# ak110/object_detector

Hardware: AMD Instinct MI355X
Metric: images_per_sec (higher is better)
Workload: dtype f16

## Files before the change

### object_detector_amd/csrc/detect.hip

```cpp
#include <string.h>

#include "post_common.h"

namespace {

constexpr int NB = OD_TOPK_NB;
constexpr int DT_ROWS = OD_DT_ROWS, DT2_RPT = OD_DT2_RPT;
constexpr int DT_CAND_CAP = 1024;

__global__ __launch_bounds__(256) void od_detect_pass1(const float* __restrict__ pred, const float* __restrict__ priors,
                                                       float* __restrict__ boxes, float* __restrict__ rowmax,
                                                       float* __restrict__ conf_out, int* __restrict__ hist,
                                                       TopkState* __restrict__ st, int P, int NC, float loc_scale, int clip,
                                                       float thr, unsigned dbase, int dshift) {
  extern __shared__ __attribute__((aligned(16))) float sm[];
  const int C = NC + 6, tid = threadIdx.x, b = blockIdx.y;
  float* rows = sm;
  int* lh = (int*)(sm + DT_ROWS * C);
  const int p0 = blockIdx.x * DT_ROWS;
  const int nrows = min(DT_ROWS, P - p0);
  for (int i = tid; i < NB; i += 256) lh[i] = 0;
  if (blockIdx.x == 0 && tid == 0) {
    TopkState z = {0, 0, 0, 0};
    st[b] = z;
  }
  const long long r0 = (long long)b * P + p0;
  const float* src = pred + r0 * C;
  const int nel = nrows * C;
  for (int i = tid * 4; i < nel; i += 256 * 4) {
    if (i + 3 < nel) {
      *(f32x4*)(rows + i) = *(const f32x4*)(src + i);
    } else {
      for (int e = i; e < nel; ++e) rows[e] = src[e];
    }
  }
  __syncthreads();
  if (tid < nrows) {
    float* row = rows + tid * C;
    const f32x4 loc = {row[2 + NC], row[3 + NC], row[4 + NC], row[5 + NC]};
    od_row_conf(row, NC, row + 2);
    float mx = 0.f;
    for (int c = 0; c < NC; ++c) {
      const float v = row[2 + c];
      mx = fmaxf(mx, v);
      const unsigned sb = od_score_bits(v, thr);
      if (sb) atomicAdd(&lh[od_digit0(sb, dbase, dshift)], 1);
    }
    rowmax[r0 + tid] = mx;
    const f32x4 pr = *(const f32x4*)(priors + (long long)(p0 + tid) * 4);
    *(f32x4*)(boxes + (r0 + tid) * 4) = od_decode_one(loc, pr, loc_scale, clip);
  }
  __syncthreads();
  int* gh = hist + (long long)b * NB;
  for (int i = tid; i < NB; i += 256)
    if (lh[i]) atomicAdd(&gh[i], lh[i]);
  if (conf_out) {
    float* dst = conf_out + r0 * NC;
    for (int i = tid; i < nrows * NC; i += 256) {
      const int r = i / NC, c = i - r * NC;
      dst[i] = rows[r * C + 2 + c];
    }
  }
}

__global__ __launch_bounds__(256) void od_detect_pass2(const float* __restrict__ pred, const float* __restrict__ rowmax,
                                                       const int* __restrict__ hist, TopkState* __restrict__ st,
                                                       u64* __restrict__ keys, u64* __restrict__ cand, int P, int NC, int K,
                                                       float thr, long long cand_stride, unsigned dbase, int dshift) {
  extern __shared__ __attribute__((aligned(16))) float sm[];
  const int C = NC + 6, tid = threadIdx.x, b = blockIdx.y;
  float* rows = sm;
  u64* l_out = (u64*)(sm + DT_ROWS * C);
  u64* l_cand = l_out + K;
  __shared__ int n_out, n_cand, n_hot, base_out, base_cand, sh_fd[8];
  __shared__ int hot_list[DT_ROWS * DT2_RPT];
  if (tid == 0) {
    n_out = 0;
    n_cand = 0;
    n_hot = 0;
  }
  int d0, above;
  od_find_digit_256(hist + (long long)b * NB, K, sh_fd, &d0, &above);
  if (blockIdx.x == 0 && tid == 0) {
    st[b].d0 = d0;
    st[b].krem = d0 < 0 ? 0 : K - above;
  }
  const int p_base = blockIdx.x * (DT_ROWS * DT2_RPT);
  const int nh = od_compact_hot_priors(rowmax + (long long)b * P, P, p_base, thr, dbase, dshift, d0, hot_list, &n_hot);
  for (int e = tid; e < nh; e += 256) {
    const int p = hot_list[e];
    float* row = rows + tid * C;
    const float* src = pred + ((long long)b * P + p) * C;
    for (int c = 0; c < 2 + NC; ++c) row[c] = src[c];
    od_row_conf(row, NC, row + 2);
    for (int c = 0; c < NC; ++c) {
      const unsigned sbc = od_score_bits(row[2 + c], thr);
      if (!sbc) continue;
      const int dg = od_digit0(sbc, dbase, dshift);
      if (dg < d0) continue;
      const unsigned flat = (unsigned)(p * NC + c);
      const u64 key = od_make_key(sbc, flat);
      if (dg > d0) {
        l_out[atomicAdd(&n_out, 1)] = key;
      } else {
        const int slot = atomicAdd(&n_cand, 1);
        if (slot < DT_CAND_CAP) {
          l_cand[slot] = key;
        } else {
          cand[(long long)b * cand_stride + atomicAdd(&st[b].ncand, 1)] = key;
        }
      }
    }
  }
  __syncthreads();
  const int nc = min(n_cand, DT_CAND_CAP);
  if (tid == 0) base_cand = nc ? atomicAdd(&st[b].ncand, nc) : 0;
  od_block_copy_out(l_out, n_out, &st[b].nout, keys + (long long)b * K, &base_out);
  u64* oc = cand + (long long)b * cand_stride + base_cand;
  for (int j = tid; j < nc; j += 256) oc[j] = l_cand[j];
}

__global__ __launch_bounds__(1024) void od_detect_refine_sort(const float* __restrict__ boxes, TopkState* __restrict__ st,
                                                              u64* __restrict__ keys, const u64* __restrict__ cand,
                                                              int* __restrict__ hist, int* __restrict__ counts, int P, int NC,
                                                              int K, int KP, long long cand_stride, u64* __restrict__ skeys,
                                                              f32x4* __restrict__ sbox, int* __restrict__ scls, unsigned dbase,
                                                              int dshift) {
  __shared__ u64 s[1024];
  __shared__ int n_win;
  const int b = blockIdx.x, tid = threadIdx.x;
  const TopkState t = st[b];
  const int nout0 = min(t.nout, K);
  if (tid == 0) n_win = 0;
  s[tid] = tid < nout0 ? keys[(long long)b * K + tid] : 0ull;
  __syncthreads();
  if (t.d0 >= 0 && t.krem > 0) {
    const u64* ic = cand + (long long)b * cand_stride;
    od_radix_refine(
        t.ncand, t.ncand, t.krem, dbase, dshift, [&](int i) { return ic[i]; },
        [&](u64 key) {
          const int slot = nout0 + atomicAdd(&n_win, 1);
          if (slot < K) s[slot] = key;
        });
    __syncthreads();
  }
  od_bitonic_sort_desc(s, KP);
  od_rank_gather(s, min(nout0 + n_win, K), b, boxes, P, NC, K, KP, skeys, sbox, scls, keys, counts, hist);
}

__global__ __launch_bounds__(256) void od_gather_det_pred(const float* __restrict__ pred, const float* __restrict__ boxes,
                                                          const int32_t* __restrict__ keep_flat,
                                                          const int32_t* __restrict__ keep_count, int P, int NC, int max_det,
                                                          float* __restrict__ out) {
  extern __shared__ __attribute__((aligned(16))) float sm[];
  const int b = blockIdx.x, C = NC + 6;
  const int n = keep_count[b];
  float* o = out + (size_t)b * (1 + 6 * (size_t)max_det);
  if (threadIdx.x == 0) o[0] = __int_as_float(n);
  float* row = sm + threadIdx.x * C;
  for (int r = threadIdx.x; r < max_det; r += 256) {
    float* rec = o + 1 + 6 * (size_t)r;
    if (r < n) {
      const int flat = keep_flat[(size_t)b * max_det + r];
      const int p = flat / NC, c = flat - p * NC;
      const float* src = pred + ((size_t)b * P + p) * C;
      for (int e = 0; e < 2 + NC; ++e) row[e] = src[e];
      od_row_conf(row, NC, row + 2);
      const float* bx = boxes + ((size_t)b * P + p) * 4;
      rec[0] = __int_as_float(flat);
      rec[1] = row[2 + c];
      rec[2] = bx[0];
      rec[3] = bx[1];
      rec[4] = bx[2];
      rec[5] = bx[3];
    } else {
      rec[0] = __int_as_float(-1);
      rec[1] = rec[2] = rec[3] = rec[4] = rec[5] = 0.f;
    }
  }
}

struct DetLayout {
  size_t hist, state, rowmax, cand, total;
  long long cand_stride;
  size_t nhot, hot;
};
DetLayout det_layout(int B, int P, int NC) {
  DetLayout l;
  size_t o = 0;
  l.hist = o;
  o += (size_t)B * NB * sizeof(int);
  l.state = o;
  o += ((size_t)B * sizeof(TopkState) + 255) & ~(size_t)255;
  l.rowmax = o;
  o += (((size_t)B * P * sizeof(float)) + 255) & ~(size_t)255;
  if (NC > OD_MAX_LDS_NC) {
    l.cand = 0;
    l.cand_stride = 0;
    l.nhot = o;
    o += ((size_t)B * sizeof(int) + 255) & ~(size_t)255;
    l.hot = o;
    o += (size_t)B * P * sizeof(HotRow);
    l.total = o;
    return l;
  }
  l.nhot = l.hot = 0;
  l.cand = o;
  l.cand_stride = (long long)P * NC;
  o += (size_t)B * (size_t)l.cand_stride * sizeof(u64);
  l.total = o;
  return l;
}

}

extern "C" size_t od_detect_workspace_bytes(int B, int P, int NC, int K) {
  (void)K;
  if (B <= 0 || P <= 0 || NC <= 0) return 0;
  return det_layout(B, P, NC).total;
}

extern "C" int od_detect_workspace_init(od_ctx* ctx, void* workspace, size_t workspace_bytes, int B, int P, int NC, void* stream) {
  OD_REQUIRE(ctx && workspace && B > 0 && P > 0 && NC > 0, "od_detect_workspace_init: bad argument");
  const DetLayout l = det_layout(B, P, NC);
  if (workspace_bytes < l.total) {
    od_set_error("od_detect_workspace_init: workspace %zu < %zu bytes", workspace_bytes, l.total);
    return OD_ERR_WORKSPACE;
  }
  OD_CHECK_HIP(hipMemsetAsync(workspace, 0, l.rowmax, (hipStream_t)stream));
  return OD_OK;
}

namespace {
int detect_candidates_launch(od_ctx* ctx, const char* who, const float* pred, const float* priors, int B, int P, int NC,
                             float loc_scale, int clip, float conf_threshold, int K, float* boxes, float* conf, uint64_t* keys,
                             int32_t* counts, void* workspace, size_t workspace_bytes, void* nms_workspace,
                             size_t nms_workspace_bytes, hipStream_t s) {
  OD_REQUIRE(NC >= 1 && NC <= OD_MAX_NC, "%s: NC = %d outside the supported class counts 1..%d", who, NC, OD_MAX_NC);
  OD_REQUIRE(B > 0 && B <= 65535 && P > 0 && P % 2 == 0 && K > 0 && K <= 1024, "%s: bad dims (P even, K <= 1024)", who);
  OD_REQUIRE((long long)P * NC < (1LL << 31), "%s: P * NC must fit 31 bits", who);
  OD_REQUIRE(conf_threshold >= 0.f, "%s: conf_threshold must be >= 0 (scores are probabilities)", who);
  const DetLayout l = det_layout(B, P, NC);
  if (workspace_bytes < l.total) {
    od_set_error("%s: workspace %zu < %zu bytes", who, workspace_bytes, l.total);
    return OD_ERR_WORKSPACE;
  }
  if (nms_workspace_bytes < od_nms_workspace_bytes(B, K)) {
    od_set_error("%s: NMS workspace %zu < %zu bytes", who, nms_workspace_bytes, od_nms_workspace_bytes(B, K));
    return OD_ERR_WORKSPACE;
  }
  char* ws = (char*)workspace;
  int* hist = (int*)(ws + l.hist);
  TopkState* st = (TopkState*)(ws + l.state);
  float* rowmax = (float*)(ws + l.rowmax);
  u64* cand = (u64*)(ws + l.cand);
  const int C = NC + 6;
  unsigned dbase;
  memcpy(&dbase, &conf_threshold, 4);
  int dshift = 0;
  while (((0x3F800000u - dbase) >> dshift) >= (unsigned)NB) ++dshift;
  const dim3 grid((unsigned)od_ceil_div(P, DT_ROWS), (unsigned)B);
  const dim3 grid2((unsigned)od_ceil_div(P, DT_ROWS * DT2_RPT), (unsigned)B);
  u64* skeys;
  f32x4* sbox;
  int* scls;
  int KP;
  od_nms_sorted_buffers(nms_workspace, B, K, &skeys, &sbox, &scls, &KP);
  if (NC > OD_MAX_LDS_NC) {
    return od_detect_wide_launch(pred, priors, B, P, NC, loc_scale, clip, conf_threshold, dbase, dshift, K, KP, boxes, conf,
                                 (u64*)keys, counts, hist, st, rowmax, (int*)(ws + l.nhot), (HotRow*)(ws + l.hot), skeys, sbox,
                                 scls, s);
  }
  const size_t lds1 = (size_t)DT_ROWS * C * 4 + (size_t)NB * 4;
  if (int rc = od_ensure_lds(ctx, (const void*)&od_detect_pass1, lds1)) return rc;
  hipLaunchKernelGGL(od_detect_pass1, grid, dim3(256), lds1, s, pred, priors, boxes, rowmax, conf, hist, st, P, NC, loc_scale,
                     clip, conf_threshold, dbase, dshift);
  OD_CHECK_LAUNCH();
  const size_t lds2 = (size_t)DT_ROWS * C * 4 + ((size_t)K + DT_CAND_CAP) * 8;
  if (int rc = od_ensure_lds(ctx, (const void*)&od_detect_pass2, lds2)) return rc;
  hipLaunchKernelGGL(od_detect_pass2, grid2, dim3(256), lds2, s, pred, rowmax, hist, st, (u64*)keys, cand, P, NC, K,
                     conf_threshold, l.cand_stride, dbase, dshift);
  OD_CHECK_LAUNCH();
  hipLaunchKernelGGL(od_detect_refine_sort, dim3(B), dim3(1024), 0, s, boxes, st, (u64*)keys, cand, hist, counts, P, NC, K, KP,
                     l.cand_stride, skeys, sbox, scls, dbase, dshift);
  OD_CHECK_LAUNCH();
  return OD_OK;
}
}

extern "C" int od_detect(od_ctx* ctx, const float* pred, const float* priors, int B, int P, int NC, float loc_scale, int clip,
                         float conf_threshold, int K, float iou_threshold, int strict, int max_det, float* boxes, float* conf,
                         uint64_t* keys, int32_t* counts, int32_t* keep_flat, int32_t* keep_count, void* workspace,
                         size_t workspace_bytes, void* nms_workspace, size_t nms_workspace_bytes, void* stream) {
  OD_REQUIRE(ctx && pred && priors && boxes && keys && counts && keep_flat && keep_count && workspace && nms_workspace,
             "od_detect: null argument");
  OD_REQUIRE(max_det > 0, "od_detect: bad dims (P even, K <= 1024)");
  hipStream_t s = (hipStream_t)stream;
  if (int rc = detect_candidates_launch(ctx, "od_detect", pred, priors, B, P, NC, loc_scale, clip, conf_threshold, K, boxes, conf,
                                        keys, counts, workspace, workspace_bytes, nms_workspace, nms_workspace_bytes, s))
    return rc;
  return od_nms_mask_scan_launch(ctx, nms_workspace, counts, B, K, iou_threshold, strict, max_det, keep_flat, keep_count, s);
}

extern "C" int od_detect_candidates(od_ctx* ctx, const float* pred, const float* priors, int B, int P, int NC, float loc_scale,
                                    int clip, float conf_threshold, int K, float* boxes, float* conf, uint64_t* keys,
                                    int32_t* counts, void* workspace, size_t workspace_bytes, void* nms_workspace,
                                    size_t nms_workspace_bytes, void* stream) {
  OD_REQUIRE(ctx && pred && priors && boxes && keys && counts && workspace && nms_workspace, "od_detect_candidates: null argument");
  return detect_candidates_launch(ctx, "od_detect_candidates", pred, priors, B, P, NC, loc_scale, clip, conf_threshold, K, boxes,
                                  conf, keys, counts, workspace, workspace_bytes, nms_workspace, nms_workspace_bytes,
                                  (hipStream_t)stream);
}

extern "C" int od_gather_detections_pred(od_ctx* ctx, const float* pred, const float* boxes, const int32_t* keep_flat,
                                         const int32_t* keep_count, int B, int P, int NC, int max_det, float* out, void* stream) {
  OD_REQUIRE(ctx && pred && boxes && keep_flat && keep_count && out, "od_gather_detections_pred: null argument");
  OD_REQUIRE(NC >= 1 && NC <= OD_MAX_NC, "od_gather_detections_pred: NC = %d outside the supported class counts 1..%d", NC,
             OD_MAX_NC);
  OD_REQUIRE(B > 0 && P > 0 && max_det > 0, "od_gather_detections_pred: bad dims");
  if (NC > OD_MAX_LDS_NC) {
    return od_gather_det_pred_wide_launch(pred, boxes, keep_flat, keep_count, B, P, NC, max_det, out, (hipStream_t)stream);
  }
  hipLaunchKernelGGL(od_gather_det_pred, dim3(B), dim3(256), (size_t)256 * (NC + 6) * 4, (hipStream_t)stream, pred, boxes,
                     keep_flat, keep_count, P, NC, max_det, out);
  OD_CHECK_LAUNCH();
  return OD_OK;
}
```

### object_detector_amd/csrc/nms.hip

```cpp
#include "post_common.h"

namespace {

__global__ __launch_bounds__(1024) void od_nms_sort(const float* __restrict__ boxes, const u64* __restrict__ keys,
                                                    const int* __restrict__ counts, int P, int NC, int K, int KP,
                                                    u64* __restrict__ skeys, f32x4* __restrict__ sbox,
                                                    int* __restrict__ scls) {
  __shared__ u64 s[1024];
  const int b = blockIdx.x, tid = threadIdx.x;
  if (tid < KP) s[tid] = tid < K ? keys[(long long)b * K + tid] : 0ull;
  __syncthreads();
  od_bitonic_sort_desc(s, KP);
  od_rank_gather(s, counts[b], b, boxes, P, NC, K, KP, skeys, sbox, scls, nullptr, nullptr, nullptr);
}

__global__ __launch_bounds__(1024) void od_nms_mask(const f32x4* __restrict__ sbox, const int* __restrict__ scls,
                                                   const int* __restrict__ counts, int KP, int W, float thr, int strict,
                                                   u64* __restrict__ mask) {
  extern __shared__ __attribute__((aligned(16))) char sm[];
  f32x4* lb = (f32x4*)sm;
  int* lc = (int*)(sm + (size_t)KP * 16);
  const int b = blockIdx.y, rb = blockIdx.x, tid = threadIdx.x, lane = tid & 63, wv = tid >> 6;
  const int n = counts[b];
  if (rb * 64 >= n) {
    for (int w = rb + wv; w < W; w += 16) mask[((long long)b * KP + rb * 64 + lane) * W + w] = 0ull;
    return;
  }
  for (int i = tid; i < n; i += 1024) {
    lb[i] = sbox[(long long)b * KP + i];
    lc[i] = scls[(long long)b * KP + i];
  }
  __syncthreads();
  const int i = rb * 64 + lane;
  const bool rowok = i < n;
  const f32x4 a = rowok ? lb[i] : f32x4{0.f, 0.f, 0.f, 0.f};
  const int ca = rowok ? lc[i] : -1;
  const float area_a = (a[2] - a[0]) * (a[3] - a[1]);
  for (int w = rb + wv; w < W; w += 16) {
    u64 bits = 0ull;
    const int jend = min(64, n - w * 64);
    for (int jj = 0; jj < jend; ++jj) {
      const int j = w * 64 + jj;
      const f32x4 c = lb[j];
      const int cc = lc[j];
      const bool hit = rowok && j > i && (strict || cc == ca) && od_iou_exceeds(a, area_a, c, thr);
      bits |= (u64)hit << jj;
    }
    mask[((long long)b * KP + i) * W + w] = bits;
  }
}

__device__ __forceinline__ u64 readlane64(u64 v, int l) {
  const unsigned lo = __builtin_amdgcn_readlane((unsigned)v, l);
  const unsigned hi = __builtin_amdgcn_readlane((unsigned)(v >> 32), l);
  return ((u64)hi << 32) | lo;
}

__global__ __launch_bounds__(256) void od_nms_scan(const u64* __restrict__ mask, const u64* __restrict__ skeys,
                                                   const int* __restrict__ counts, int KP, int W, int max_det,
                                                   int* __restrict__ keep_flat, int* __restrict__ keep_count) {
  extern __shared__ __attribute__((aligned(16))) u64 lm[];
  const int b = blockIdx.x, tid = threadIdx.x, lane = tid & 63;
  const int n = __builtin_amdgcn_readfirstlane(counts[b]);
  const u64* mb = mask + (long long)b * KP * W;
  for (int i = tid; i < n * W; i += 256) lm[i] = mb[i];
  __syncthreads();
  if (tid >= 64) return;
  u64* keptw = lm + (size_t)KP * W;

  const int w = lane & 15, g = lane >> 4;
  u64 removed = 0ull;
#pragma unroll 1
  for (int blk = 0; blk < W; ++blk) {
    u64 alive = 0ull;
    if (blk * 64 < n) {
      const int nv = n - blk * 64;
      const u64 valid = nv >= 64 ? ~0ull : ((1ull << nv) - 1ull);
      alive = ~readlane64(removed, blk) & valid;
      const u64 dg = (lane < nv) ? lm[(size_t)(blk * 64 + lane) * W + blk] : 0ull;
      u64 todo = __ballot(dg != 0ull) & alive;
      while (todo) {
        const int r = __builtin_ctzll(todo);
        todo &= todo - 1ull;
        if ((alive >> r) & 1ull) {
          alive &= ~readlane64(dg, r);
          todo &= alive;
        }
      }
      u64 acc = 0ull;
      const bool wok = w < W && w > blk;
#pragma unroll
      for (int t = 0; t < 16; ++t) {
        const int r = t * 4 + g;
        const bool on = wok && ((alive >> r) & 1ull);
        const u64 v = on ? lm[(size_t)(blk * 64 + r) * W + w] : 0ull;
        acc |= v;
      }
      acc |= __shfl_xor(acc, 16);
      acc |= __shfl_xor(acc, 32);
      removed |= acc;
    }
    if (lane == 0) keptw[blk] = alive;
  }
  __builtin_amdgcn_s_waitcnt(0xC07F);
  int base = 0;
  for (int blk = 0; blk < W; ++blk) {
    const u64 kw = keptw[blk];
    const int pos = base + __popcll(kw & ((1ull << lane) - 1ull));
    if (((kw >> lane) & 1ull) && pos < max_det) {
      const u64 key = skeys[(long long)b * KP + blk * 64 + lane];
      keep_flat[(long long)b * max_det + pos] = (int)od_key_flat(key);
    }
    base += __popcll(kw);
  }
  const int total = min(base, max_det);
  for (int i = total + lane; i < max_det; i += 64) keep_flat[(long long)b * max_det + i] = -1;
  if (lane == 0) keep_count[b] = total;
}

int next_pow2(int v) {
  int p = 64;
  while (p < v) p <<= 1;
  return p;
}

struct NmsLayout {
  size_t skeys, sbox, scls, mask, total;
};
NmsLayout nms_layout(int B, int KP) {
  NmsLayout l;
  size_t o = 0;
  l.skeys = o;
  o += (size_t)B * KP * 8;
  l.sbox = o;
  o += (size_t)B * KP * 16;
  l.scls = o;
  o += (size_t)B * KP * 4;
  l.mask = o;
  o += (size_t)B * KP * (KP / 64) * 8;
  l.total = o;
  return l;
}

}

void od_nms_sorted_buffers(void* nms_workspace, int B, int K, unsigned long long** skeys, f32x4** sbox, int** scls, int* KP) {
  const int kp = next_pow2(K);
  const NmsLayout l = nms_layout(B, kp);
  char* ws = (char*)nms_workspace;
  *skeys = (unsigned long long*)(ws + l.skeys);
  *sbox = (f32x4*)(ws + l.sbox);
  *scls = (int*)(ws + l.scls);
  *KP = kp;
}

int od_nms_mask_scan_launch(od_ctx* ctx, void* nms_workspace, const int32_t* counts, int B, int K, float iou_threshold,
                            int strict, int max_det, int32_t* keep_flat, int32_t* keep_count, hipStream_t s) {
  const int KP = next_pow2(K), W = KP / 64;
  const NmsLayout l = nms_layout(B, KP);
  char* ws = (char*)nms_workspace;
  u64* skeys = (u64*)(ws + l.skeys);
  f32x4* sbox = (f32x4*)(ws + l.sbox);
  int* scls = (int*)(ws + l.scls);
  u64* mask = (u64*)(ws + l.mask);
  hipLaunchKernelGGL(od_nms_mask, dim3(W, B), dim3(1024), (size_t)KP * 20, s, sbox, scls, counts, KP, W, iou_threshold,
                     strict, mask);
  OD_CHECK_LAUNCH();
  const size_t scan_lds = (size_t)KP * W * 8 + 16 * 8;
  if (int rc = od_ensure_lds(ctx, (const void*)&od_nms_scan, scan_lds)) return rc;
  hipLaunchKernelGGL(od_nms_scan, dim3(B), dim3(256), scan_lds, s, mask, skeys, counts, KP, W, max_det, keep_flat,
                     keep_count);
  OD_CHECK_LAUNCH();
  return OD_OK;
}

extern "C" size_t od_nms_workspace_bytes(int B, int K) {
  if (B <= 0 || K <= 0 || K > 1024) return 0;
  return nms_layout(B, next_pow2(K)).total;
}

extern "C" int od_nms(od_ctx* ctx, const float* boxes, const uint64_t* keys, const int32_t* counts, int B, int P, int NC,
                      int K, float iou_threshold, int strict, int max_det, int32_t* keep_flat, int32_t* keep_count,
                      void* workspace, size_t workspace_bytes, void* stream) {
  OD_REQUIRE(ctx && boxes && keys && counts && keep_flat && keep_count && workspace, "od_nms: null argument");
  OD_REQUIRE(B > 0 && B <= 65535 && P > 0 && NC > 0 && K > 0 && K <= 1024 && max_det > 0,
             "od_nms: bad dims (K <= 1024)");
  const int KP = next_pow2(K);
  const NmsLayout l = nms_layout(B, KP);
  if (workspace_bytes < l.total) {
    od_set_error("od_nms: workspace %zu < %zu bytes", workspace_bytes, l.total);
    return OD_ERR_WORKSPACE;
  }
  char* ws = (char*)workspace;
  u64* skeys = (u64*)(ws + l.skeys);
  f32x4* sbox = (f32x4*)(ws + l.sbox);
  int* scls = (int*)(ws + l.scls);
  hipStream_t s = (hipStream_t)stream;
  hipLaunchKernelGGL(od_nms_sort, dim3(B), dim3(1024), 0, s, boxes, (const u64*)keys, counts, P, NC, K, KP, skeys, sbox,
                     scls);
  OD_CHECK_LAUNCH();
  return od_nms_mask_scan_launch(ctx, workspace, counts, B, K, iou_threshold, strict, max_det, keep_flat, keep_count, s);
}
```

### object_detector_amd/csrc/post_common.h

```cpp
#pragma once
#include "common.h"

constexpr int OD_TOPK_NB = 4096;

struct TopkState {
  int d0;
  int krem;
  int nout;
  int ncand;
};

__device__ __forceinline__ void od_row_conf(const float* row, int NC, float* out) {
  const float obj = 1.f / (1.f + expf(row[0] - row[1]));
  float mx = row[2];
  for (int c = 1; c < NC; ++c) mx = fmaxf(mx, row[2 + c]);
  float s = 0.f;
  for (int c = 0; c < NC; ++c) {
    const float e = expf(row[2 + c] - mx);
    out[c] = e;
    s += e;
  }
  for (int c = 0; c < NC; ++c) out[c] = obj * (out[c] / s);
}

// ... 115 lines not shown
}

__device__ __forceinline__ int od_find_digit(const int* hist, int nbins, int krem, int* above, int* in_bin) {
  const int lane = threadIdx.x & 63;
  const int per = nbins / 64;
  int s = 0;
  for (int i = 0; i < per; ++i) s += hist[lane * per + i];
  int suf = s;
#pragma unroll
  for (int off = 1; off < 64; off <<= 1) {
    const int o = __shfl_down(suf, off);
    if (lane + off < 64) suf += o;
  }
  const int higher = suf - s;
  const bool mine = higher < krem && suf >= krem;
  const unsigned long long bal = __ballot(mine);
  int digit = -1, ab = 0, ib = 0;
  if (bal) {
    const int owner = __ffsll((long long)bal) - 1;
    if (lane == owner) {
      int run = higher;
      for (int i = per - 1; i >= 0; --i) {
        const int c = hist[lane * per + i];
        if (run + c >= krem) {
          digit = lane * per + i;
          ab = run;
          ib = c;
          break;
        }
        run += c;
      }
    }
    digit = __shfl(digit, owner);
    ab = __shfl(ab, owner);
    ib = __shfl(ib, owner);
  }
  *above = ab;
  *in_bin = ib;
  return digit;
}

#include "topk_common.h"

struct HotRow {
  int p;
  OdRowStats r;
};
int od_detect_wide_launch(const float* pred, const float* priors, int B, int P, int NC, float loc_scale, int clip, float thr,
                          unsigned dbase, int dshift, int K, int KP, float* boxes, float* conf, unsigned long long* keys,
                          int* counts, int* hist, TopkState* st, float* rowmax, int* nhot, HotRow* hot,
                          unsigned long long* skeys, f32x4* sbox, int* scls, hipStream_t s);
int od_gather_det_pred_wide_launch(const float* pred, const float* boxes, const int32_t* keep_flat, const int32_t* keep_count,
                                   int B, int P, int NC, int max_det, float* out, hipStream_t s);
int od_nms_mask_scan_launch(od_ctx* ctx, void* nms_workspace, const int32_t* counts, int B, int K, float iou_threshold,
                            int strict, int max_det, int32_t* keep_flat, int32_t* keep_count, hipStream_t stream);
void od_nms_sorted_buffers(void* nms_workspace, int B, int K, unsigned long long** skeys, f32x4** sbox, int** scls, int* KP);
```

### object_detector_amd/csrc/topk_common.h

```cpp
#pragma once

typedef unsigned long long u64;

__device__ __forceinline__ u64 od_make_key(unsigned score_bits, unsigned flat) {
  return ((u64)score_bits << 32) | (u64)(0xFFFFFFFFu - flat);
}
__device__ __forceinline__ unsigned od_key_flat(u64 key) { return 0xFFFFFFFFu - (unsigned)key; }
__device__ __forceinline__ unsigned od_key_score_bits(u64 key) { return (unsigned)(key >> 32); }

__device__ __forceinline__ u64 od_refine_subkey(u64 key, unsigned dbase, unsigned low_mask) {
  return ((u64)((od_key_score_bits(key) - dbase) & low_mask) << 32) | (key & 0xFFFFFFFFull);
}

template <class KeyAt, class Emit>
__device__ __forceinline__ void od_radix_refine(int n, int nc, int krem, unsigned dbase, int dshift, KeyAt key_at, Emit emit) {
  __shared__ int lh[OD_TOPK_NB];
  __shared__ int sh_digit, sh_above, sh_inbin;
  const int tid = threadIdx.x;
  const unsigned low_mask = (1u << dshift) - 1u;
  u64 prefix = 0, pmask = 0;
  const int shifts[5] = {40, 32, 21, 10, 0};
  const int widths[5] = {11, 8, 11, 11, 10};
  bool whole = (nc == krem);
  for (int ps = 0; ps < 5 && !whole; ++ps) {
    const int sh = shifts[ps], nbins = 1 << widths[ps];
    for (int i = tid; i < OD_TOPK_NB; i += 1024) lh[i] = 0;
    __syncthreads();
    for (int i = tid; i < n; i += 1024) {
      const u64 key = key_at(i);
      if (!key) continue;
      const u64 sub = od_refine_subkey(key, dbase, low_mask);
      if ((sub & pmask) == prefix) atomicAdd(&lh[(int)((sub >> sh) & (u64)(nbins - 1))], 1);
    }
    __syncthreads();
    if (tid < 64) {
      int above, in_bin;
      const int d = od_find_digit(lh, OD_TOPK_NB, krem, &above, &in_bin);
      if (tid == 0) {
        sh_digit = d;
        sh_above = above;
        sh_inbin = in_bin;
      }
    }
    __syncthreads();
    prefix |= (u64)sh_digit << sh;
    pmask |= (u64)(nbins - 1) << sh;
    krem -= sh_above;
    whole = (sh_inbin == krem);
    __syncthreads();
  }
  for (int i = tid; i < n; i += 1024) {
    const u64 key = key_at(i);
    if (key && (od_refine_subkey(key, dbase, low_mask) & pmask) >= prefix) emit(key);
  }
}

__device__ __forceinline__ void od_bitonic_sort_desc(u64* s, int KP) {
  const int tid = threadIdx.x;
  for (int k = 2; k <= KP; k <<= 1) {
    for (int j = k >> 1; j > 0; j >>= 1) {
      const int ixj = tid ^ j;
      if (tid < KP && ixj > tid) {
        const u64 a = s[tid], c = s[ixj];
        const bool desc = (tid & k) == 0;
        if (desc ? (a < c) : (a > c)) {
          s[tid] = c;
          s[ixj] = a;
        }
      }
      __syncthreads();
    }
  }
}

__device__ __forceinline__ void od_rank_gather(const u64* s, int n, int b, const float* __restrict__ boxes, int P, int NC, int K,
                                               int KP, u64* __restrict__ skeys, f32x4* __restrict__ sbox, int* __restrict__ scls,
                                               u64* __restrict__ keys, int* __restrict__ counts, int* __restrict__ hist) {
  const int tid = threadIdx.x;
  if (tid < KP) {
    const u64 key = s[tid];
    skeys[(long long)b * KP + tid] = key;
    if (keys && tid < K) keys[(long long)b * K + tid] = key;
    if (tid < n) {
      const unsigned flat = od_key_flat(key);
      const unsigned p = flat / (unsigned)NC;
      const unsigned c = flat - p * (unsigned)NC;
      sbox[(long long)b * KP + tid] = *(const f32x4*)(boxes + ((long long)b * P + p) * 4);
      scls[(long long)b * KP + tid] = (int)c;
    }
  }
  if (counts && tid == 0) counts[b] = n;
  if (hist) {
    int* gh = hist + (long long)b * OD_TOPK_NB;
    for (int i = tid; i < OD_TOPK_NB; i += 1024) gh[i] = 0;
  }
}

constexpr int OD_DT_ROWS = 256;
constexpr int OD_DT2_RPT = 4;

__device__ __forceinline__ int od_compact_hot_priors(const float* __restrict__ rowmax_b, int P, int p_base, float thr,
                                                     unsigned dbase, int dshift, int d0, int* hot_list, int* n_hot) {
  const int tid = threadIdx.x;
  float mxv[OD_DT2_RPT];
#pragma unroll
  for (int u = 0; u < OD_DT2_RPT; ++u) {
    const int p = p_base + u * OD_DT_ROWS + tid;
    mxv[u] = p < P ? rowmax_b[p] : 0.f;
  }
#pragma unroll
  for (int u = 0; u < OD_DT2_RPT; ++u) {
    const unsigned sb = od_score_bits(mxv[u], thr);
    if (sb && od_digit0(sb, dbase, dshift) >= d0) hot_list[atomicAdd(n_hot, 1)] = p_base + u * OD_DT_ROWS + tid;
  }
  __syncthreads();
  return *n_hot;
}

__device__ __forceinline__ void od_block_copy_out(const u64* l, int n, int* total, u64* __restrict__ dst, int* sh_base) {
  const int tid = threadIdx.x;
  if (tid == 0) *sh_base = n ? atomicAdd(total, n) : 0;
  __syncthreads();
  u64* o = dst + *sh_base;
  for (int j = tid; j < n; j += 256) o[j] = l[j];
}

__device__ __forceinline__ bool od_iou_exceeds(const f32x4 a, float area_a, const f32x4 c, float thr) {
  const float ix1 = fmaxf(a[0], c[0]), iy1 = fmaxf(a[1], c[1]);
  const float ix2 = fminf(a[2], c[2]), iy2 = fminf(a[3], c[3]);
  const float iw = fmaxf(ix2 - ix1, 0.f), ih = fmaxf(iy2 - iy1, 0.f);
  const float inter = iw * ih;
  const float area_c = (c[2] - c[0]) * (c[3] - c[1]);
  const float uni = (area_a + area_c) - inter;
  return inter > thr * uni;
}
```

### object_detector_amd/csrc/tta.hip

```cpp
#include "post_common.h"

namespace {

constexpr int TTA_MAX_VIEWS = 8;
constexpr int TTA_MAX_K = 1024;

struct TtaViews {
  const u64* keys[TTA_MAX_VIEWS];
  const int* counts[TTA_MAX_VIEWS];
  const float* boxes[TTA_MAX_VIEWS];
  int P[TTA_MAX_VIEWS];
  int flip[TTA_MAX_VIEWS];
  int V;
};

__global__ __launch_bounds__(256) void od_hflip_u8_x16(const uint4* __restrict__ src, uint4* __restrict__ dst, int gpr,
                                                       long long ngroups) {
  for (long long g = (long long)blockIdx.x * 256 + threadIdx.x; g < ngroups; g += (long long)gridDim.x * 256) {
    const long long row = g / gpr;
    const int gx = (int)(g - row * gpr);
    const long long sg = row * gpr + (gpr - 1 - gx);
    const uint4 a = src[sg * 3], b = src[sg * 3 + 1], c = src[sg * 3 + 2];
    const unsigned in[12] = {a.x, a.y, a.z, a.w, b.x, b.y, b.z, b.w, c.x, c.y, c.z, c.w};
    unsigned o[12];
// ... 214 lines not shown
    const long long ngroups = npix / 16;
    const unsigned grid = (unsigned)((ngroups + 255) / 256 < 4096 ? (ngroups + 255) / 256 : 4096);
    hipLaunchKernelGGL(od_hflip_u8_x16, dim3(grid), dim3(256), 0, s, (const uint4*)src, (uint4*)dst, W / 16, ngroups);
  } else {
    const unsigned grid = (unsigned)((npix + 255) / 256 < 4096 ? (npix + 255) / 256 : 4096);
    hipLaunchKernelGGL(od_hflip_u8_px, dim3(grid), dim3(256), 0, s, src, dst, W, npix);
  }
  OD_CHECK_LAUNCH();
  return OD_OK;
}

extern "C" size_t od_tta_merge_workspace_bytes(int B, int V, int K) {
  if (B <= 0 || V < 1 || V > TTA_MAX_VIEWS || K <= 0 || K > TTA_MAX_K) return 0;
  return tta_layout(B, K).total;
}

extern "C" int od_tta_merge(od_ctx* ctx, const od_tta_view* views, int V, int B, int NC, int K, float iou_threshold,
                            int strict, int max_det, float vote_iou, float* out, int32_t* src, int32_t* keep_count,
                            void* workspace, size_t workspace_bytes, void* stream) {
  OD_REQUIRE(ctx && views && out && keep_count && workspace, "od_tta_merge: null argument");
  OD_REQUIRE(V >= 1 && V <= TTA_MAX_VIEWS, "od_tta_merge: V = %d outside 1..%d", V, TTA_MAX_VIEWS);
  OD_REQUIRE(NC >= 1 && NC <= OD_MAX_NC, "od_tta_merge: NC = %d outside the supported class counts 1..%d", NC, OD_MAX_NC);
  OD_REQUIRE(B > 0 && B <= 65535 && K > 0 && K <= TTA_MAX_K && max_det > 0, "od_tta_merge: bad dims (K <= 1024)");
  TtaViews vw = {};
  vw.V = V;
  for (int v = 0; v < V; ++v) {
    OD_REQUIRE(views[v].keys && views[v].counts && views[v].boxes, "od_tta_merge: view %d has a null pointer", v);
    OD_REQUIRE(views[v].P > 0 && (long long)views[v].P * NC < (1LL << 31), "od_tta_merge: view %d: P * NC must fit 31 bits", v);
    vw.keys[v] = (const u64*)views[v].keys;
    vw.counts[v] = views[v].counts;
    vw.boxes[v] = views[v].boxes;
    vw.P[v] = views[v].P;
    vw.flip[v] = views[v].flip != 0;
  }
  const TtaLayout l = tta_layout(B, K);
  if (workspace_bytes < l.total) {
    od_set_error("od_tta_merge: workspace %zu < %zu bytes", workspace_bytes, l.total);
    return OD_ERR_WORKSPACE;
  }
  char* ws = (char*)workspace;
  void* nms_ws = ws + l.nms;
  int* mcount = (int*)(ws + l.mcount);
  int* msrc = (int*)(ws + l.msrc);
  int* keepf = (int*)(ws + l.keepf);
  u64* skeys;
  f32x4* sbox;
  int* scls;
  int KP;
  od_nms_sorted_buffers(nms_ws, B, K, &skeys, &sbox, &scls, &KP);
  hipStream_t s = (hipStream_t)stream;
  hipLaunchKernelGGL(od_tta_merge_rank, dim3(B), dim3(1024), 0, s, vw, NC, K, KP, skeys, sbox, scls, msrc, mcount);
  OD_CHECK_LAUNCH();
  const int md = max_det < K ? max_det : K;
  if (int rc = od_nms_mask_scan_launch(ctx, nms_ws, mcount, B, K, iou_threshold, strict, md, keepf, keep_count, s)) return rc;
  hipLaunchKernelGGL(od_tta_vote_gather, dim3(B), dim3(1024), 0, s, skeys, sbox, scls, msrc, mcount, keepf, keep_count, NC, KP, md,
                     max_det, vote_iou, out, src);
  OD_CHECK_LAUNCH();
  return OD_OK;
}
```

Before: 22120.

## Fuse refine-sort with greedy blockwise NMS and specialize pass1 staging

Replaces the two-kernel NMS (full IoU bitmask plus a scan) with a single-block greedy NMS that tests each 64-column chunk only against boxes already kept plus the chunk's own diagonal. For the standard detect path this NMS is fused into the refine/sort kernel, with sorted boxes kept in LDS. Pass1 also gains an odd row pitch to avoid LDS bank conflicts, alignment-dependent vector staging, and an NC=20 template specialization that keeps confidences in registers. The goal is fewer launches, less mask memory traffic and faster pass1, at the cost of a serial per-chunk dependency inside one block per image.

```diff
diff --git a/object_detector_amd/csrc/detect.hip b/object_detector_amd/csrc/detect.hip
--- a/object_detector_amd/csrc/detect.hip
+++ b/object_detector_amd/csrc/detect.hip
@@ -8,15 +8,46 @@
 constexpr int DT_ROWS = OD_DT_ROWS, DT2_RPT = OD_DT2_RPT;
 constexpr int DT_CAND_CAP = 1024;
 
+constexpr int dt_row_pitch(int C) { return C | 1; }
+
+template <int V>
+__device__ __forceinline__ void dt_stage_rows(const float* __restrict__ src, int nel, int C, int CS, float* rows) {
+  typedef float vec __attribute__((ext_vector_type(V)));
+  constexpr int U = 8;
+  const int nfull = nel & ~(V - 1);
+  const int step = 256 * V, dr = step / C, dc = step - dr * C;
+  int i = threadIdx.x * V, r = i / C, c = i - r * C;
+  for (; i < nfull; i += U * step) {
+    vec t[U];
+#pragma unroll
+    for (int u = 0; u < U; ++u) t[u] = *(const vec*)(src + min(i + u * step, nfull - V));
+#pragma unroll
+    for (int u = 0; u < U; ++u) {
+      int rr = r, cc = c;
+#pragma unroll
+      for (int e = 0; e < V; ++e) {
+        if (i + u * step < nfull) rows[rr * CS + cc] = t[u][e];
+        if (++cc == C) cc = 0, ++rr;
+      }
+      r += dr, c += dc;
+      if (c >= C) c -= C, ++r;
+    }
+  }
+  const int e = nfull + threadIdx.x;
+  if (e < nel) rows[(e / C) * CS + (e - (e / C) * C)] = src[e];
+}
+
+template <int NCT>
 __global__ __launch_bounds__(256) void od_detect_pass1(const float* __restrict__ pred, const float* __restrict__ priors,
                                                        float* __restrict__ boxes, float* __restrict__ rowmax,
                                                        float* __restrict__ conf_out, int* __restrict__ hist,
-                                                       TopkState* __restrict__ st, int P, int NC, float loc_scale, int clip,
+                                                       TopkState* __restrict__ st, int P, int NC_rt, float loc_scale, int clip,
                                                        float thr, unsigned dbase, int dshift) {
   extern __shared__ __attribute__((aligned(16))) float sm[];
-  const int C = NC + 6, tid = threadIdx.x, b = blockIdx.y;
+  const int NC = NCT ? NCT : NC_rt;
+  const int C = NC + 6, CS = dt_row_pitch(C), tid = threadIdx.x, b = blockIdx.y;
   float* rows = sm;
-  int* lh = (int*)(sm + DT_ROWS * C);
+  int* lh = (int*)(sm + DT_ROWS * CS);
   const int p0 = blockIdx.x * DT_ROWS;
   const int nrows = min(DT_ROWS, P - p0);
   for (int i = tid; i < NB; i += 256) lh[i] = 0;
@@ -27,24 +58,36 @@
   const long long r0 = (long long)b * P + p0;
   const float* src = pred + r0 * C;
   const int nel = nrows * C;
-  for (int i = tid * 4; i < nel; i += 256 * 4) {
-    if (i + 3 < nel) {
-      *(f32x4*)(rows + i) = *(const f32x4*)(src + i);
-    } else {
-      for (int e = i; e < nel; ++e) rows[e] = src[e];
-    }
+  const unsigned mis = (unsigned)(uintptr_t)src & 15u;
+  if (mis == 0) {
+    dt_stage_rows<4>(src, nel, C, CS, rows);
+  } else if ((mis & 7u) == 0) {
+    dt_stage_rows<2>(src, nel, C, CS, rows);
+  } else {
+    dt_stage_rows<1>(src, nel, C, CS, rows);
   }
   __syncthreads();
   if (tid < nrows) {
-    float* row = rows + tid * C;
+    float* row = rows + tid * CS;
     const f32x4 loc = {row[2 + NC], row[3 + NC], row[4 + NC], row[5 + NC]};
-    od_row_conf(row, NC, row + 2);
     float mx = 0.f;
-    for (int c = 0; c < NC; ++c) {
-      const float v = row[2 + c];
+    const auto score = [&](float v) {
       mx = fmaxf(mx, v);
       const unsigned sb = od_score_bits(v, thr);
       if (sb) atomicAdd(&lh[od_digit0(sb, dbase, dshift)], 1);
+    };
+    if constexpr (NCT > 0) {
+      float cf[NCT];
+      od_row_conf(row, NCT, cf);
+#pragma unroll
+      for (int c = 0; c < NCT; ++c) score(cf[c]);
+      if (conf_out) {
+#pragma unroll
+        for (int c = 0; c < NCT; ++c) row[2 + c] = cf[c];
+      }
+    } else {
+      od_row_conf(row, NC, row + 2);
+      for (int c = 0; c < NC; ++c) score(row[2 + c]);
     }
     rowmax[r0 + tid] = mx;
     const f32x4 pr = *(const f32x4*)(priors + (long long)(p0 + tid) * 4);
@@ -58,7 +101,7 @@
     float* dst = conf_out + r0 * NC;
     for (int i = tid; i < nrows * NC; i += 256) {
       const int r = i / NC, c = i - r * NC;
-      dst[i] = rows[r * C + 2 + c];
+      dst[i] = rows[r * CS + 2 + c];
     }
   }
 }
@@ -120,32 +163,60 @@
   for (int j = tid; j < nc; j += 256) oc[j] = l_cand[j];
 }
 
-__global__ __launch_bounds__(1024) void od_detect_refine_sort(const float* __restrict__ boxes, TopkState* __restrict__ st,
-                                                              u64* __restrict__ keys, const u64* __restrict__ cand,
-                                                              int* __restrict__ hist, int* __restrict__ counts, int P, int NC,
-                                                              int K, int KP, long long cand_stride, u64* __restrict__ skeys,
-                                                              f32x4* __restrict__ sbox, int* __restrict__ scls, unsigned dbase,
-                                                              int dshift) {
-  __shared__ u64 s[1024];
+struct RefineArgs {
+  const float* boxes;
+  TopkState* st;
+  u64* keys;
+  const u64* cand;
+  int *hist, *counts;
+  int P, NC, K, KP;
+  long long cand_stride;
+  u64* skeys;
+  f32x4* sbox;
+  int* scls;
+  unsigned dbase;
+  int dshift;
+};
+
+__device__ __forceinline__ int dt_refine_sort_gather(const RefineArgs& a, u64* s, f32x4* lbox, int* lcls) {
   __shared__ int n_win;
-  const int b = blockIdx.x, tid = threadIdx.x;
-  const TopkState t = st[b];
+  const int b = blockIdx.x, tid = threadIdx.x, K = a.K;
+  const TopkState t = a.st[b];
   const int nout0 = min(t.nout, K);
   if (tid == 0) n_win = 0;
-  s[tid] = tid < nout0 ? keys[(long long)b * K + tid] : 0ull;
+  s[tid] = tid < nout0 ? a.keys[(long long)b * K + tid] : 0ull;
   __syncthreads();
   if (t.d0 >= 0 && t.krem > 0) {
-    const u64* ic = cand + (long long)b * cand_stride;
+    const u64* ic = a.cand + (long long)b * a.cand_stride;
     od_radix_refine(
-        t.ncand, t.ncand, t.krem, dbase, dshift, [&](int i) { return ic[i]; },
+        t.ncand, t.ncand, t.krem, a.dbase, a.dshift, [&](int i) { return ic[i]; },
         [&](u64 key) {
           const int slot = nout0 + atomicAdd(&n_win, 1);
           if (slot < K) s[slot] = key;
         });
     __syncthreads();
   }
-  od_bitonic_sort_desc(s, KP);
-  od_rank_gather(s, min(nout0 + n_win, K), b, boxes, P, NC, K, KP, skeys, sbox, scls, keys, counts, hist);
+  od_bitonic_sort_desc(s, a.KP);
+  const int n = min(nout0 + n_win, K);
+  od_rank_gather(s, n, b, a.boxes, a.P, a.NC, K, a.KP, a.skeys, a.sbox, a.scls, a.keys, a.counts, a.hist, lbox, lcls);
+  return n;
+}
+
+__global__ __launch_bounds__(1024) void od_detect_refine_sort(const RefineArgs a) {
+  __shared__ u64 s[1024];
+  dt_refine_sort_gather(a, s, nullptr, nullptr);
+}
+
+__global__ __launch_bounds__(1024) void od_detect_tail(const RefineArgs a, float iou_thr, int strict, int max_det,
+                                                       int* __restrict__ keep_flat, int* __restrict__ keep_count) {
+  extern __shared__ __attribute__((aligned(16))) char smem[];
+  u64* s = (u64*)smem;
+  f32x4* lb = (f32x4*)(smem + 1024 * 8);
+  int* lc = (int*)(lb + a.KP);
+  const int b = blockIdx.x;
+  const int n = dt_refine_sort_gather(a, s, lb, lc);
+  __syncthreads();
+  od_nms_greedy(lb, lc, s, n, iou_thr, strict, max_det, keep_flat + (long long)b * max_det, keep_count + b);
 }
 
 __global__ __launch_bounds__(256) void od_gather_det_pred(const float* __restrict__ pred, const float* __restrict__ boxes,
@@ -232,10 +303,27 @@
 }
 
 namespace {
-int detect_candidates_launch(od_ctx* ctx, const char* who, const float* pred, const float* priors, int B, int P, int NC,
-                             float loc_scale, int clip, float conf_threshold, int K, float* boxes, float* conf, uint64_t* keys,
-                             int32_t* counts, void* workspace, size_t workspace_bytes, void* nms_workspace,
-                             size_t nms_workspace_bytes, hipStream_t s) {
+struct NmsArgs {
+  float iou_threshold;
+  int strict, max_det;
+  int32_t *keep_flat, *keep_count;
+};
+
+template <int NCT>
+int launch_pass1(od_ctx* ctx, dim3 grid, size_t lds, hipStream_t s, const float* pred, const float* priors, float* boxes,
+                 float* rowmax, float* conf, int* hist, TopkState* st, int P, int NC, float loc_scale, int clip, float thr,
+                 unsigned dbase, int dshift) {
+  if (int rc = od_ensure_lds(ctx, (const void*)&od_detect_pass1<NCT>, lds)) return rc;
+  hipLaunchKernelGGL(od_detect_pass1<NCT>, grid, dim3(256), lds, s, pred, priors, boxes, rowmax, conf, hist, st, P, NC, loc_scale,
+                     clip, thr, dbase, dshift);
+  OD_CHECK_LAUNCH();
+  return OD_OK;
+}
+
+int detect_launch(od_ctx* ctx, const char* who, const float* pred, const float* priors, int B, int P, int NC, float loc_scale,
+                  int clip, float conf_threshold, int K, float* boxes, float* conf, uint64_t* keys, int32_t* counts,
+                  void* workspace, size_t workspace_bytes, void* nms_workspace, size_t nms_workspace_bytes, const NmsArgs* nms,
+                  hipStream_t s) {
   OD_REQUIRE(NC >= 1 && NC <= OD_MAX_NC, "%s: NC = %d outside the supported class counts 1..%d", who, NC, OD_MAX_NC);
   OD_REQUIRE(B > 0 && B <= 65535 && P > 0 && P % 2 == 0 && K > 0 && K <= 1024, "%s: bad dims (P even, K <= 1024)", who);
   OD_REQUIRE((long long)P * NC < (1LL << 31), "%s: P * NC must fit 31 bits", who);
@@ -267,22 +355,32 @@
   int KP;
   od_nms_sorted_buffers(nms_workspace, B, K, &skeys, &sbox, &scls, &KP);
   if (NC > OD_MAX_LDS_NC) {
-    return od_detect_wide_launch(pred, priors, B, P, NC, loc_scale, clip, conf_threshold, dbase, dshift, K, KP, boxes, conf,
-                                 (u64*)keys, counts, hist, st, rowmax, (int*)(ws + l.nhot), (HotRow*)(ws + l.hot), skeys, sbox,
-                                 scls, s);
-  }
-  const size_t lds1 = (size_t)DT_ROWS * C * 4 + (size_t)NB * 4;
-  if (int rc = od_ensure_lds(ctx, (const void*)&od_detect_pass1, lds1)) return rc;
-  hipLaunchKernelGGL(od_detect_pass1, grid, dim3(256), lds1, s, pred, priors, boxes, rowmax, conf, hist, st, P, NC, loc_scale,
-                     clip, conf_threshold, dbase, dshift);
-  OD_CHECK_LAUNCH();
+    if (int rc = od_detect_wide_launch(pred, priors, B, P, NC, loc_scale, clip, conf_threshold, dbase, dshift, K, KP, boxes, conf,
+                                       (u64*)keys, counts, hist, st, rowmax, (int*)(ws + l.nhot), (HotRow*)(ws + l.hot), skeys,
+                                       sbox, scls, s))
+      return rc;
+    if (!nms) return OD_OK;
+    return od_nms_greedy_launch(nms_workspace, counts, B, K, nms->iou_threshold, nms->strict, nms->max_det, nms->keep_flat,
+                                nms->keep_count, s);
+  }
+  const size_t lds1 = (size_t)DT_ROWS * dt_row_pitch(C) * 4 + (size_t)NB * 4;
+  const auto pass1 = NC == 20 ? launch_pass1<20> : launch_pass1<0>;
+  if (int rc = pass1(ctx, grid, lds1, s, pred, priors, boxes, rowmax, conf, hist, st, P, NC, loc_scale, clip, conf_threshold,
+                     dbase, dshift))
+    return rc;
   const size_t lds2 = (size_t)DT_ROWS * C * 4 + ((size_t)K + DT_CAND_CAP) * 8;
   if (int rc = od_ensure_lds(ctx, (const void*)&od_detect_pass2, lds2)) return rc;
   hipLaunchKernelGGL(od_detect_pass2, grid2, dim3(256), lds2, s, pred, rowmax, hist, st, (u64*)keys, cand, P, NC, K,
                      conf_threshold, l.cand_stride, dbase, dshift);
   OD_CHECK_LAUNCH();
-  hipLaunchKernelGGL(od_detect_refine_sort, dim3(B), dim3(1024), 0, s, boxes, st, (u64*)keys, cand, hist, counts, P, NC, K, KP,
-                     l.cand_stride, skeys, sbox, scls, dbase, dshift);
+  const RefineArgs ra = {boxes, st, (u64*)keys, cand, hist, counts, P, NC, K, KP, l.cand_stride, skeys, sbox, scls, dbase, dshift};
+  if (!nms) {
+    hipLaunchKernelGGL(od_detect_refine_sort, dim3(B), dim3(1024), 0, s, ra);
+    OD_CHECK_LAUNCH();
+    return OD_OK;
+  }
+  hipLaunchKernelGGL(od_detect_tail, dim3(B), dim3(1024), (size_t)1024 * 8 + (size_t)KP * 20, s, ra, nms->iou_threshold,
+                     nms->strict, nms->max_det, nms->keep_flat, nms->keep_count);
   OD_CHECK_LAUNCH();
   return OD_OK;
 }
@@ -295,11 +393,9 @@
   OD_REQUIRE(ctx && pred && priors && boxes && keys && counts && keep_flat && keep_count && workspace && nms_workspace,
              "od_detect: null argument");
   OD_REQUIRE(max_det > 0, "od_detect: bad dims (P even, K <= 1024)");
-  hipStream_t s = (hipStream_t)stream;
-  if (int rc = detect_candidates_launch(ctx, "od_detect", pred, priors, B, P, NC, loc_scale, clip, conf_threshold, K, boxes, conf,
-                                        keys, counts, workspace, workspace_bytes, nms_workspace, nms_workspace_bytes, s))
-    return rc;
-  return od_nms_mask_scan_launch(ctx, nms_workspace, counts, B, K, iou_threshold, strict, max_det, keep_flat, keep_count, s);
+  const NmsArgs nms = {iou_threshold, strict, max_det, keep_flat, keep_count};
+  return detect_launch(ctx, "od_detect", pred, priors, B, P, NC, loc_scale, clip, conf_threshold, K, boxes, conf, keys, counts,
+                       workspace, workspace_bytes, nms_workspace, nms_workspace_bytes, &nms, (hipStream_t)stream);
 }
 
 extern "C" int od_detect_candidates(od_ctx* ctx, const float* pred, const float* priors, int B, int P, int NC, float loc_scale,
@@ -307,9 +403,8 @@
                                     int32_t* counts, void* workspace, size_t workspace_bytes, void* nms_workspace,
                                     size_t nms_workspace_bytes, void* stream) {
   OD_REQUIRE(ctx && pred && priors && boxes && keys && counts && workspace && nms_workspace, "od_detect_candidates: null argument");
-  return detect_candidates_launch(ctx, "od_detect_candidates", pred, priors, B, P, NC, loc_scale, clip, conf_threshold, K, boxes,
-                                  conf, keys, counts, workspace, workspace_bytes, nms_workspace, nms_workspace_bytes,
-                                  (hipStream_t)stream);
+  return detect_launch(ctx, "od_detect_candidates", pred, priors, B, P, NC, loc_scale, clip, conf_threshold, K, boxes, conf, keys,
+                       counts, workspace, workspace_bytes, nms_workspace, nms_workspace_bytes, nullptr, (hipStream_t)stream);
 }
 
 extern "C" int od_gather_detections_pred(od_ctx* ctx, const float* pred, const float* boxes, const int32_t* keep_flat,
diff --git a/object_detector_amd/csrc/nms.hip b/object_detector_amd/csrc/nms.hip
--- a/object_detector_amd/csrc/nms.hip
+++ b/object_detector_amd/csrc/nms.hip
@@ -14,108 +14,23 @@
   od_rank_gather(s, counts[b], b, boxes, P, NC, K, KP, skeys, sbox, scls, nullptr, nullptr, nullptr);
 }
 
-__global__ __launch_bounds__(1024) void od_nms_mask(const f32x4* __restrict__ sbox, const int* __restrict__ scls,
-                                                   const int* __restrict__ counts, int KP, int W, float thr, int strict,
-                                                   u64* __restrict__ mask) {
+__global__ __launch_bounds__(1024) void od_nms_greedy_k(const u64* __restrict__ skeys, const f32x4* __restrict__ sbox,
+                                                       const int* __restrict__ scls, const int* __restrict__ counts, int KP,
+                                                       float thr, int strict, int max_det, int* __restrict__ keep_flat,
+                                                       int* __restrict__ keep_count) {
   extern __shared__ __attribute__((aligned(16))) char sm[];
   f32x4* lb = (f32x4*)sm;
-  int* lc = (int*)(sm + (size_t)KP * 16);
-  const int b = blockIdx.y, rb = blockIdx.x, tid = threadIdx.x, lane = tid & 63, wv = tid >> 6;
-  const int n = counts[b];
-  if (rb * 64 >= n) {
-    for (int w = rb + wv; w < W; w += 16) mask[((long long)b * KP + rb * 64 + lane) * W + w] = 0ull;
-    return;
-  }
-  for (int i = tid; i < n; i += 1024) {
-    lb[i] = sbox[(long long)b * KP + i];
-    lc[i] = scls[(long long)b * KP + i];
+  u64* lk = (u64*)(lb + KP);
+  int* lc = (int*)(lk + KP);
+  const int b = blockIdx.x, tid = threadIdx.x;
+  const int n = min(counts[b], KP);
+  if (tid < n) {
+    lb[tid] = sbox[(long long)b * KP + tid];
+    lk[tid] = skeys[(long long)b * KP + tid];
+    lc[tid] = scls[(long long)b * KP + tid];
   }
   __syncthreads();
-  const int i = rb * 64 + lane;
-  const bool rowok = i < n;
-  const f32x4 a = rowok ? lb[i] : f32x4{0.f, 0.f, 0.f, 0.f};
-  const int ca = rowok ? lc[i] : -1;
-  const float area_a = (a[2] - a[0]) * (a[3] - a[1]);
-  for (int w = rb + wv; w < W; w += 16) {
-    u64 bits = 0ull;
-    const int jend = min(64, n - w * 64);
-    for (int jj = 0; jj < jend; ++jj) {
-      const int j = w * 64 + jj;
-      const f32x4 c = lb[j];
-      const int cc = lc[j];
-      const bool hit = rowok && j > i && (strict || cc == ca) && od_iou_exceeds(a, area_a, c, thr);
-      bits |= (u64)hit << jj;
-    }
-    mask[((long long)b * KP + i) * W + w] = bits;
-  }
-}
-
-__device__ __forceinline__ u64 readlane64(u64 v, int l) {
-  const unsigned lo = __builtin_amdgcn_readlane((unsigned)v, l);
-  const unsigned hi = __builtin_amdgcn_readlane((unsigned)(v >> 32), l);
-  return ((u64)hi << 32) | lo;
-}
-
-__global__ __launch_bounds__(256) void od_nms_scan(const u64* __restrict__ mask, const u64* __restrict__ skeys,
-                                                   const int* __restrict__ counts, int KP, int W, int max_det,
-                                                   int* __restrict__ keep_flat, int* __restrict__ keep_count) {
-  extern __shared__ __attribute__((aligned(16))) u64 lm[];
-  const int b = blockIdx.x, tid = threadIdx.x, lane = tid & 63;
-  const int n = __builtin_amdgcn_readfirstlane(counts[b]);
-  const u64* mb = mask + (long long)b * KP * W;
-  for (int i = tid; i < n * W; i += 256) lm[i] = mb[i];
-  __syncthreads();
-  if (tid >= 64) return;
-  u64* keptw = lm + (size_t)KP * W;
-
-  const int w = lane & 15, g = lane >> 4;
-  u64 removed = 0ull;
-#pragma unroll 1
-  for (int blk = 0; blk < W; ++blk) {
-    u64 alive = 0ull;
-    if (blk * 64 < n) {
-      const int nv = n - blk * 64;
-      const u64 valid = nv >= 64 ? ~0ull : ((1ull << nv) - 1ull);
-      alive = ~readlane64(removed, blk) & valid;
-      const u64 dg = (lane < nv) ? lm[(size_t)(blk * 64 + lane) * W + blk] : 0ull;
-      u64 todo = __ballot(dg != 0ull) & alive;
-      while (todo) {
-        const int r = __builtin_ctzll(todo);
-        todo &= todo - 1ull;
-        if ((alive >> r) & 1ull) {
-          alive &= ~readlane64(dg, r);
-          todo &= alive;
-        }
-      }
-      u64 acc = 0ull;
-      const bool wok = w < W && w > blk;
-#pragma unroll
-      for (int t = 0; t < 16; ++t) {
-        const int r = t * 4 + g;
-        const bool on = wok && ((alive >> r) & 1ull);
-        const u64 v = on ? lm[(size_t)(blk * 64 + r) * W + w] : 0ull;
-        acc |= v;
-      }
-      acc |= __shfl_xor(acc, 16);
-      acc |= __shfl_xor(acc, 32);
-      removed |= acc;
-    }
-    if (lane == 0) keptw[blk] = alive;
-  }
-  __builtin_amdgcn_s_waitcnt(0xC07F);
-  int base = 0;
-  for (int blk = 0; blk < W; ++blk) {
-    const u64 kw = keptw[blk];
-    const int pos = base + __popcll(kw & ((1ull << lane) - 1ull));
-    if (((kw >> lane) & 1ull) && pos < max_det) {
-      const u64 key = skeys[(long long)b * KP + blk * 64 + lane];
-      keep_flat[(long long)b * max_det + pos] = (int)od_key_flat(key);
-    }
-    base += __popcll(kw);
-  }
-  const int total = min(base, max_det);
-  for (int i = total + lane; i < max_det; i += 64) keep_flat[(long long)b * max_det + i] = -1;
-  if (lane == 0) keep_count[b] = total;
+  od_nms_greedy(lb, lc, lk, n, thr, strict, max_det, keep_flat + (long long)b * max_det, keep_count + b);
 }
 
 int next_pow2(int v) {
@@ -154,21 +69,13 @@
   *KP = kp;
 }
 
-int od_nms_mask_scan_launch(od_ctx* ctx, void* nms_workspace, const int32_t* counts, int B, int K, float iou_threshold,
-                            int strict, int max_det, int32_t* keep_flat, int32_t* keep_count, hipStream_t s) {
-  const int KP = next_pow2(K), W = KP / 64;
+int od_nms_greedy_launch(void* nms_workspace, const int32_t* counts, int B, int K, float iou_threshold, int strict, int max_det,
+                         int32_t* keep_flat, int32_t* keep_count, hipStream_t s) {
+  const int KP = next_pow2(K);
   const NmsLayout l = nms_layout(B, KP);
   char* ws = (char*)nms_workspace;
-  u64* skeys = (u64*)(ws + l.skeys);
-  f32x4* sbox = (f32x4*)(ws + l.sbox);
-  int* scls = (int*)(ws + l.scls);
-  u64* mask = (u64*)(ws + l.mask);
-  hipLaunchKernelGGL(od_nms_mask, dim3(W, B), dim3(1024), (size_t)KP * 20, s, sbox, scls, counts, KP, W, iou_threshold,
-                     strict, mask);
-  OD_CHECK_LAUNCH();
-  const size_t scan_lds = (size_t)KP * W * 8 + 16 * 8;
-  if (int rc = od_ensure_lds(ctx, (const void*)&od_nms_scan, scan_lds)) return rc;
-  hipLaunchKernelGGL(od_nms_scan, dim3(B), dim3(256), scan_lds, s, mask, skeys, counts, KP, W, max_det, keep_flat,
+  hipLaunchKernelGGL(od_nms_greedy_k, dim3(B), dim3(1024), (size_t)KP * 28, s, (const u64*)(ws + l.skeys),
+                     (const f32x4*)(ws + l.sbox), (const int*)(ws + l.scls), counts, KP, iou_threshold, strict, max_det, keep_flat,
                      keep_count);
   OD_CHECK_LAUNCH();
   return OD_OK;
@@ -199,5 +106,5 @@
   hipLaunchKernelGGL(od_nms_sort, dim3(B), dim3(1024), 0, s, boxes, (const u64*)keys, counts, P, NC, K, KP, skeys, sbox,
                      scls);
   OD_CHECK_LAUNCH();
-  return od_nms_mask_scan_launch(ctx, workspace, counts, B, K, iou_threshold, strict, max_det, keep_flat, keep_count, s);
+  return od_nms_greedy_launch(workspace, counts, B, K, iou_threshold, strict, max_det, keep_flat, keep_count, s);
 }
diff --git a/object_detector_amd/csrc/post_common.h b/object_detector_amd/csrc/post_common.h
--- a/object_detector_amd/csrc/post_common.h
+++ b/object_detector_amd/csrc/post_common.h
@@ -191,6 +191,6 @@
                           unsigned long long* skeys, f32x4* sbox, int* scls, hipStream_t s);
 int od_gather_det_pred_wide_launch(const float* pred, const float* boxes, const int32_t* keep_flat, const int32_t* keep_count,
                                    int B, int P, int NC, int max_det, float* out, hipStream_t s);
-int od_nms_mask_scan_launch(od_ctx* ctx, void* nms_workspace, const int32_t* counts, int B, int K, float iou_threshold,
-                            int strict, int max_det, int32_t* keep_flat, int32_t* keep_count, hipStream_t stream);
+int od_nms_greedy_launch(void* nms_workspace, const int32_t* counts, int B, int K, float iou_threshold, int strict, int max_det,
+                         int32_t* keep_flat, int32_t* keep_count, hipStream_t stream);
 void od_nms_sorted_buffers(void* nms_workspace, int B, int K, unsigned long long** skeys, f32x4** sbox, int** scls, int* KP);
diff --git a/object_detector_amd/csrc/topk_common.h b/object_detector_amd/csrc/topk_common.h
--- a/object_detector_amd/csrc/topk_common.h
+++ b/object_detector_amd/csrc/topk_common.h
@@ -75,7 +75,8 @@
 
 __device__ __forceinline__ void od_rank_gather(const u64* s, int n, int b, const float* __restrict__ boxes, int P, int NC, int K,
                                                int KP, u64* __restrict__ skeys, f32x4* __restrict__ sbox, int* __restrict__ scls,
-                                               u64* __restrict__ keys, int* __restrict__ counts, int* __restrict__ hist) {
+                                               u64* __restrict__ keys, int* __restrict__ counts, int* __restrict__ hist,
+                                               f32x4* lbox = nullptr, int* lcls = nullptr) {
   const int tid = threadIdx.x;
   if (tid < KP) {
     const u64 key = s[tid];
@@ -85,8 +86,13 @@
       const unsigned flat = od_key_flat(key);
       const unsigned p = flat / (unsigned)NC;
       const unsigned c = flat - p * (unsigned)NC;
-      sbox[(long long)b * KP + tid] = *(const f32x4*)(boxes + ((long long)b * P + p) * 4);
+      const f32x4 box = *(const f32x4*)(boxes + ((long long)b * P + p) * 4);
+      sbox[(long long)b * KP + tid] = box;
       scls[(long long)b * KP + tid] = (int)c;
+      if (lbox) {
+        lbox[tid] = box;
+        lcls[tid] = (int)c;
+      }
     }
   }
   if (counts && tid == 0) counts[b] = n;
@@ -134,3 +140,80 @@
   const float uni = (area_a + area_c) - inter;
   return inter > thr * uni;
 }
+
+__device__ __forceinline__ bool od_suppresses(const f32x4 a, int ca, const f32x4 c, int cc, float thr, int strict) {
+  const float area_a = (a[2] - a[0]) * (a[3] - a[1]);
+  return (strict || cc == ca) && od_iou_exceeds(a, area_a, c, thr);
+}
+
+__device__ __forceinline__ u64 od_readlane64(u64 v, int l) {
+  const unsigned lo = __builtin_amdgcn_readlane((unsigned)v, l);
+  const unsigned hi = __builtin_amdgcn_readlane((unsigned)(v >> 32), l);
+  return ((u64)hi << 32) | lo;
+}
+
+__device__ __forceinline__ void od_nms_greedy(const f32x4* lb, const int* lc, const u64* skeys, int n, float thr, int strict,
+                                              int max_det, int* __restrict__ keep_flat, int* __restrict__ keep_count) {
+  __shared__ int kept[1024];
+  __shared__ u64 dgw[64];
+  __shared__ u64 remw;
+  __shared__ int nkept;
+  const int tid = threadIdx.x, lane = tid & 63, wv = tid >> 6;
+  if (tid == 0) {
+    remw = 0ull;
+    nkept = 0;
+  }
+  __syncthreads();
+  const int W = (n + 63) >> 6;
+  int total = 0;
+  for (int blk = 0; blk < W && total < max_det; ++blk) {
+    const int j = blk * 64 + lane;
+    const bool colok = j < n;
+    const f32x4 c = colok ? lb[j] : f32x4{0.f, 0.f, 0.f, 0.f};
+    const int cc = colok ? lc[j] : -1;
+    bool rem = false;
+    for (int e = wv; e < total; e += 16) {
+      const int r = kept[e];
+      rem |= colok && od_suppresses(lb[r], lc[r], c, cc, thr, strict);
+    }
+    const u64 rw = __ballot(rem);
+    if (lane == 0 && rw) atomicOr((u64*)&remw, rw);
+#pragma unroll
+    for (int q = 0; q < 4; ++q) {
+      const int rr = wv * 4 + q, i = blk * 64 + rr;
+      const bool hit = i < n && colok && j > i && od_suppresses(lb[i], lc[i], c, cc, thr, strict);
+      const u64 wd = __ballot(hit);
+      if (lane == 0) dgw[rr] = wd;
+    }
+    __syncthreads();
+    if (wv == 0) {
+      const int nv = n - blk * 64;
+      const u64 valid = nv >= 64 ? ~0ull : ((1ull << nv) - 1ull);
+      u64 alive = ~remw & valid;
+      const u64 dg = dgw[lane];
+      u64 todo = __ballot(dg != 0ull) & alive;
+      while (todo) {
+        const int r = __builtin_ctzll(todo);
+        todo &= todo - 1ull;
+        if ((alive >> r) & 1ull) {
+          alive &= ~od_readlane64(dg, r);
+          todo &= alive;
+        }
+      }
+      const int pos = total + __popcll(alive & ((1ull << lane) - 1ull));
+      if ((alive >> lane) & 1ull) {
+        kept[pos] = j;
+        if (pos < max_det) keep_flat[pos] = (int)od_key_flat(skeys[j]);
+      }
+      if (lane == 0) {
+        nkept = total + __popcll(alive);
+        remw = 0ull;
+      }
+    }
+    __syncthreads();
+    total = __builtin_amdgcn_readfirstlane(nkept);
+  }
+  total = min(total, max_det);
+  for (int i = total + tid; i < max_det; i += 1024) keep_flat[i] = -1;
+  if (tid == 0) *keep_count = total;
+}
diff --git a/object_detector_amd/csrc/tta.hip b/object_detector_amd/csrc/tta.hip
--- a/object_detector_amd/csrc/tta.hip
+++ b/object_detector_amd/csrc/tta.hip
@@ -290,7 +290,7 @@
   hipLaunchKernelGGL(od_tta_merge_rank, dim3(B), dim3(1024), 0, s, vw, NC, K, KP, skeys, sbox, scls, msrc, mcount);
   OD_CHECK_LAUNCH();
   const int md = max_det < K ? max_det : K;
-  if (int rc = od_nms_mask_scan_launch(ctx, nms_ws, mcount, B, K, iou_threshold, strict, md, keepf, keep_count, s)) return rc;
+  if (int rc = od_nms_greedy_launch(nms_ws, mcount, B, K, iou_threshold, strict, md, keepf, keep_count, s)) return rc;
   hipLaunchKernelGGL(od_tta_vote_gather, dim3(B), dim3(1024), 0, s, skeys, sbox, scls, msrc, mcount, keepf, keep_count, NC, KP, md,
                      max_det, vote_iou, out, src);
   OD_CHECK_LAUNCH();
```

New measurement: 22640 (median of 6 runs). 2.3% higher.
